# dgrzech/ir-sgmcmc

Hardware: AMD Instinct MI355X
Metric: SG-MCMC transitions/sec (full _SGLD_transition) (higher is better)
Workload: dtype f32; 1 GPU; 256^3 synthetic pair, SVF_3D 12 steps, GMM(K=4)/LCC(s=1) + virtual decimation, RegLoss_L2 w=1.4, Sobolev s=3, uniform noise 0.1, SGLD lr 0.4, Philox noise; init=identity, chains=1, parallelism=1 independent chain(s)

## Files before the change

include/irsgmcmc.h:

```cpp
#ifndef IRSGMCMC_H
#define IRSGMCMC_H

#include <stddef.h>
#include <stdint.h>

#ifdef __cplusplus
extern "C" {
#endif
#pragma GCC visibility push(default)

#define IRS_MAX_COMPONENTS 8
#define IRS_MAX_CHAINS 8
#define IRS_MAX_HALF_WIDTH 4
#define IRS_MAX_LABELS 64
#define IRS_HAUSDORFF_MAX_PERCENTILES 4

enum { IRS_DATA_GMM_LCC = 0, IRS_DATA_SSD = 1 };
enum { IRS_REG_L2 = 0, IRS_REG_LOGNORMAL = 1, IRS_REG_STUDENT = 2, IRS_REG_LOGNORMAL_L2 = 3 };


int irs_perturb_smooth(const float* v, const float* sigma, const float* eps, float tau, const float* kernel, int s,
                       int C, int D, int H, int W, float* tmp, float* out, uint64_t seed, uint64_t iteration,
                       void* stream);

// ... 306 lines not shown
int irs_set_fixed(irs_ctx* ctx, const float* fixed_im, int fixed_chains, void* stream);
int irs_get_state(irs_ctx* ctx, irs_state* out, void* stream);
int irs_set_state(irs_ctx* ctx, const irs_state* in, void* stream);
int irs_get_scalars(irs_ctx* ctx, irs_scalars* out, void* stream);

int irs_gmm_init(irs_ctx* ctx, const irs_io* io, const float* v_sample, int warm_up, void* stream);

int irs_transition(irs_ctx* ctx, const irs_io* io, void* stream);

int irs_flush(irs_ctx* ctx, void* stream);
int irs_recovered_transitions(const irs_ctx* ctx, uint64_t* out);
int irs_sparse_adjoint_set(irs_ctx* ctx, int on);
int irs_sparse_adjoint_get(irs_ctx* ctx, int32_t* out, void* stream);
int irs_sparse_data_set(irs_ctx* ctx, int on);
int irs_sparse_data_get(irs_ctx* ctx, int32_t* out, void* stream);

typedef struct irs_timings {
    float total_ms;
    float exp_fwd_ms;
    float exp_bwd_kernel_ms;
    float exp_bwd_total_ms;
    float smooth_ms;
    float data_ms;
    float update_ms;
    float exp_bwd_primary_avg_ms;
} irs_timings;
int irs_transition_timed(irs_ctx* ctx, const irs_io* io, void* stream, irs_timings* out);

typedef struct irs_comm irs_comm;
#define IRS_COMM_ID_BYTES 128
// ... 95 lines not shown
```

ir_sgmcmc_amd/_lib.py:

```python
import ctypes as C
import os

import torch

_HERE = os.path.dirname(os.path.abspath(__file__))
LIB_PATH = os.environ.get('IRS_LIB') or os.path.join(_HERE, 'csrc', 'libirsgmcmc.so')

IRS_MAX_COMPONENTS = 8
IRS_MAX_CHAINS = 8
IRS_MAX_HALF_WIDTH = 4
IRS_MAX_LABELS = 64
IRS_HAUSDORFF_MAX_PERCENTILES = 4
IRS_LABEL_BINS = 10
IRS_JACOBIAN_SUMMARY_INTS, IRS_JACOBIAN_SUMMARY_FLOATS = 4, 5
IRS_JACOBIAN_WS_BYTES = 1024 * (IRS_JACOBIAN_SUMMARY_INTS + IRS_JACOBIAN_SUMMARY_FLOATS) * 8
IRS_COVARIANCE_SUMMARY_INTS, IRS_COVARIANCE_SUMMARY_FLOATS = 2, 8
IRS_COVARIANCE_WS_BYTES = 1024 * (IRS_COVARIANCE_SUMMARY_INTS + IRS_COVARIANCE_SUMMARY_FLOATS) * 8
IRS_COMPARE_SUMMARY_INTS, IRS_COMPARE_SUMMARY_FLOATS = 4, 13
IRS_COMPARE_WS_BYTES = 1024 * (IRS_COMPARE_SUMMARY_INTS + IRS_COMPARE_SUMMARY_FLOATS) * 8
IRS_QUANTILE_MIN_BINS, IRS_QUANTILE_MAX_BINS, IRS_QUANTILE_MAX_PROBS, IRS_QUANTILE_MAX_RECORDS = 4, 256, 8, 65535
IRS_QUANTILE_SUMMARY_INTS, IRS_QUANTILE_SUMMARY_FLOATS = 3, 5
IRS_QUANTILE_WS_BYTES = 1024 * (IRS_QUANTILE_SUMMARY_INTS + IRS_QUANTILE_SUMMARY_FLOATS) * 8
IRS_ICE_SUMMARY_INTS, IRS_ICE_SUMMARY_FLOATS = 2, 3
IRS_ICE_WS_BYTES = IRS_MAX_CHAINS * 1024 * (IRS_ICE_SUMMARY_INTS + IRS_ICE_SUMMARY_FLOATS) * 8
# ... 195 lines not shown
    'irs_destroy': [_P],
    'irs_workspace_bytes': [_P],
    'irs_velocity_dims': [_P, C.POINTER(C.c_int32 * 3)],
    'irs_set_fixed': [_P, _P, _I, _P],
    'irs_get_state': [_P, C.POINTER(IrsState), _P],
    'irs_set_state': [_P, C.POINTER(IrsState), _P],
    'irs_get_scalars': [_P, C.POINTER(IrsScalars), _P],
    'irs_gmm_init': [_P, C.POINTER(IrsIO), _P, _I, _P],
    'irs_transition': [_P, C.POINTER(IrsIO), _P],
    'irs_flush': [_P, _P],
    'irs_recovered_transitions': [_P, C.POINTER(C.c_uint64)],
    'irs_sparse_adjoint_set': [_P, _I],
    'irs_sparse_adjoint_get': [_P, _I32P, _P],
    'irs_sparse_data_set': [_P, _I],
    'irs_sparse_data_get': [_P, _I32P, _P],
    'irs_transition_timed': [_P, C.POINTER(IrsIO), _P, C.POINTER(IrsTimings)],
    'irs_comm_unique_id': [C.POINTER(C.c_uint8 * IRS_COMM_ID_BYTES)],
    'irs_comm_create_rccl': [C.POINTER(C.c_uint8 * IRS_COMM_ID_BYTES), _I, _I, C.POINTER(_P)],
    'irs_comm_create_ipc': [C.c_char_p, _I, _I, C.POINTER(_P)],
    'irs_comm_create_callbacks': [EXCHANGE_FN, ALLREDUCE_FN, _P, _I, _I, C.POINTER(_P)],
    'irs_comm_destroy': [_P],
    'irs_comm_probe': [_P, C.c_size_t, C.c_size_t, _I, _P, C.POINTER(C.c_double * 2)],
    'irs_comm_describe': [_P, C.c_char_p, C.c_size_t],
    'irs_comm_rank': [_P],
    'irs_comm_world': [_P],
    'irs_comm_selftest': [_P, _P],
    'irs_slab_plan_layout': [C.POINTER(IrsConfig), C.POINTER(IrsSlabConfig), _I, _I, C.POINTER(IrsSlabLayout)],
    'irs_slab_create': [C.POINTER(IrsConfig), C.POINTER(IrsSlabConfig), _P, C.POINTER(_P)],
    'irs_slab_get_layout': [_P, C.POINTER(IrsSlabLayout)],
    'irs_slab_transition': [_P, C.POINTER(IrsIO), _P],
# ... 65 lines not shown
```

ir_sgmcmc_amd/csrc/adjoint_plan.hip:

```cpp
#include "adjoint_plan.h"

#include "kernels.h"

namespace irs {

constexpr int kExtChunk = 32;

template <typename T>
__device__ __forceinline__ void extent_body(const T* __restrict__ g, int* __restrict__ ext, const Vol& vol) {
    const int x = (int)blockIdx.x * 64 + ((int)threadIdx.x & 63), y = (int)blockIdx.y * 4 + ((int)threadIdx.x >> 6);
    const int nch = (vol.D + kExtChunk - 1) / kExtChunk;
    const int chain = (int)blockIdx.z / nch, za = ((int)blockIdx.z - chain * nch) * kExtChunk, zb = min(za + kExtChunk, vol.D);
    if (x >= vol.W || y >= vol.H) return;
    const int64_t plane = (int64_t)vol.H * vol.W;
    const T* __restrict__ p = g + (int64_t)chain * vol.V + (int64_t)y * vol.W + x;
    int lo = vol.D, hi = -1;
#pragma unroll 8
    for (int z = za; z < zb; ++z) {
        const bool nz = p[z * plane] != (T)0;
        lo = nz ? min(lo, z) : lo;
        hi = nz ? z : hi;
    }
    if (hi < 0) return;
    int* e = ext + ((int64_t)chain * plane + (int64_t)y * vol.W + x) * 2;
    atomicMax(e, vol.D - lo);
    atomicMax(e + 1, hi + 1);
}
__global__ __launch_bounds__(kBlock) void grad_extent_kernel(const float* __restrict__ g, int* __restrict__ ext, Vol vol) {
    extent_body<float>(g, ext, vol);
}
__global__ __launch_bounds__(kBlock) void mask_extent_kernel(const uint8_t* __restrict__ mask, int* __restrict__ ext, Vol vol) {
    extent_body<uint8_t>(mask, ext, vol);
}
static void launch_extent(const float* g, const uint8_t* mask, int* ext, int chains, Vol vol, hipStream_t st) {
    (void)hipMemsetAsync(ext, 0, sizeof(int) * 2 * (size_t)chains * vol.H * vol.W, st);
    const int nch = (vol.D + kExtChunk - 1) / kExtChunk;
    const dim3 grid((unsigned)((vol.W + 63) / 64), (unsigned)((vol.H + 3) / 4), (unsigned)(nch * chains));
    if (g) hipLaunchKernelGGL(grad_extent_kernel, grid, dim3(kBlock), 0, st, g, ext, vol);
    else hipLaunchKernelGGL(mask_extent_kernel, grid, dim3(kBlock), 0, st, mask, ext, vol);
}

__device__ __forceinline__ bool chain_is_dense(const unsigned* __restrict__ dmax, int chain, int C, int no_steps) {
    bool dense = false;
    if (!dmax) return false;
    for (int k = 0; k < no_steps; ++k) {
        const unsigned* b = dmax + ((int64_t)k * C + chain) * 4;
        const float m = fmaxf(fmaxf(__uint_as_float(b[0]), __uint_as_float(b[1])), __uint_as_float(b[2]));
        dense |= !(m < 1.0f);
    }
    return dense;
}

__global__ __launch_bounds__(kWave) void plan_runs_kernel(const int* __restrict__ ext, int ext_chains, const unsigned* __restrict__ dmax,
                                                          int* __restrict__ runs, Vol vol, int C, int no_steps, int ntx, int nty,
                                                          PlanShape shape) {
// ... 118 lines not shown
        count[2 * k] = min(base, cap);
        count[2 * k + 1] = min(s_nrun, cap);
    }
    if (tid < C) {
        int* s = stats + ((int64_t)k * C + tid) * kPlanStats;
        s[0] = chain_is_dense(dmax, tid, C, no_steps) ? 0 : 1;
        s[1] = L;
        s[2] = s_pieces[tid];
        s[3] = s_planes[tid];
    }
}

static size_t plan_align(size_t b) { return (b + 255) / 256 * 256; }

struct PlanLayout {
    size_t ext, runs, colplan, entries, count, stats, total;
    int cap, ntx, nty;
};
static PlanLayout plan_layout(Vol vol, int C, int no_steps) {
    PlanLayout l;
    l.ntx = (vol.W + kPlanTX - 1) / kPlanTX;
    l.nty = (vol.H + kPlanTY - 1) / kPlanTY;
    const size_t cols = (size_t)C * l.ntx * l.nty;
    l.cap = plan_entries_cap((int)cols, vol.D);
    size_t off = 0;
    auto take = [&](size_t bytes) { const size_t o = off; off += plan_align(bytes); return o; };
    l.ext = take(sizeof(int) * 2 * (size_t)C * vol.H * vol.W);
    l.runs = take(sizeof(int) * 2 * cols * no_steps);
    l.colplan = take(sizeof(ColPlan) * cols * no_steps);
    l.entries = take(sizeof(PlanEntry) * (size_t)l.cap * no_steps);
    l.count = take(sizeof(int) * 2 * no_steps);
    l.stats = take(sizeof(int) * kPlanStats * (size_t)C * no_steps);
    l.total = off;
    return l;
}

size_t adjoint_plan_bytes(Vol vol, int C, int no_steps) { return plan_layout(vol, C, no_steps).total; }

AdjointPlan adjoint_plan_views(char* base, Vol vol, int C, int no_steps) {
    const PlanLayout l = plan_layout(vol, C, no_steps);
    AdjointPlan p;
    p.ext = (int*)(base + l.ext);
    p.runs = (int*)(base + l.runs);
    p.colplan = (ColPlan*)(base + l.colplan);
    p.entries = (PlanEntry*)(base + l.entries);
    p.count = (int*)(base + l.count);
    p.stats = (int*)(base + l.stats);
    p.cap = l.cap;
    p.ntx = l.ntx;
    p.nty = l.nty;
    return p;
}

void launch_adjoint_plan(const float* g_warped, const unsigned* dmax, const AdjointPlan& plan, int no_steps, int C, Vol vol,
                         int64_t G, int forced_len, hipStream_t st) {
    const int g = (int)(G > 0 ? G : 1024);
    const PlanShape shape{kPlanTX, kPlanTY, no_steps, 1, {kFillNext, kFillNext}, {g, g}, kPlanMinLen};
    launch_extent(g_warped, nullptr, plan.ext, C, vol, st);
    hipLaunchKernelGGL(plan_runs_kernel, dim3((unsigned)(C * plan.ntx * plan.nty), (unsigned)no_steps), dim3(kWave), 0, st, plan.ext, C, dmax,
                       plan.runs, vol, C, no_steps, plan.ntx, plan.nty, shape);
    hipLaunchKernelGGL(plan_lists_kernel, dim3((unsigned)no_steps), dim3(kPlanBlock), 0, st, plan.runs, dmax, plan.colplan, plan.entries, plan.count,
                       plan.stats, vol, C, no_steps, plan.ntx, plan.nty, plan.cap, shape, forced_len);
}

struct DataLayout {
    size_t ext, runs, hull, colplan, entries, count, stats, nll, total;
    int cap, ntx, nty, wtx, wty;
};
static DataLayout data_layout(Vol vol, int C) {
    DataLayout l;
    l.ntx = (vol.W + kLccTX - 1) / kLccTX;
    l.nty = (vol.H + kLccTY - 1) / kLccTY;
    l.wtx = (vol.W + kWarpTX - 1) / kWarpTX;
    l.wty = (vol.H + kWarpTY - 1) / kWarpTY;
// ... 31 lines not shown
    p.nty = l.nty;
    p.wtx = l.wtx;
    p.wty = l.wty;
    return p;
}

static int data_list_resident(int s, bool bwd, int C) {
    const int64_t res = lcc_plan_resident(s, bwd, bwd && C > 1);
    return (int)(res > 0 ? res : 1024);
}
int data_plan_run_bound(const DataPlan& plan, int s, bool bwd, int C, Vol vol) {
    return plan_run_bound(C * plan.ntx * plan.nty, vol.D, data_list_resident(s, bwd, C), plan.forced_len);
}

void launch_data_plan(const uint8_t* mask, int mask_chains, const DataPlan& plan, int s, bool lists, int C, Vol vol, hipStream_t st) {
    launch_extent(nullptr, mask, plan.ext, mask_chains, vol, st);
    const PlanShape warp{kWarpTX, kWarpTY, 3 * s, 0, {kFillNone, kFillNone}, {1, 1}, kPlanMinLen};
    hipLaunchKernelGGL(plan_runs_kernel, dim3((unsigned)(C * plan.wtx * plan.wty), 1u), dim3(kWave), 0, st, plan.ext, mask_chains, nullptr,
                       plan.hull, vol, C, 1, plan.wtx, plan.wty, warp);
    if (!lists) return;
    const PlanShape lcc{kLccTX, kLccTY, 2 * s, s, {kFillAll, kFillNone}, {data_list_resident(s, true, C), data_list_resident(s, false, C)},
                        kPlanMinLen};
    hipLaunchKernelGGL(plan_runs_kernel, dim3((unsigned)(C * plan.ntx * plan.nty), 2u), dim3(kWave), 0, st, plan.ext, mask_chains, nullptr,
                       plan.runs, vol, C, 2, plan.ntx, plan.nty, lcc);
    hipLaunchKernelGGL(plan_lists_kernel, dim3(2u), dim3(kPlanBlock), 0, st, plan.runs, nullptr, plan.colplan, plan.entries, plan.count, plan.stats,
                       vol, C, 2, plan.ntx, plan.nty, plan.cap, lcc, plan.forced_len);
}

}
```

ir_sgmcmc_amd/csrc/api_ctx.hip:

```cpp
#include <math.h>
#include <string.h>

#include <new>

#include "adjoint_plan.h"
#include "api_checks.h"
#include "comm.h"

using namespace irs;

static size_t align_up(size_t x) { return (x + 255) & ~(size_t)255; }

static bool is_capturing(hipStream_t st) {
    hipStreamCaptureStatus cap = hipStreamCaptureStatusNone;
    (void)hipStreamIsCapturing(st, &cap);
    return cap != hipStreamCaptureStatusNone;
}


int irs::create_ctx(const irs_config* cfg, const SlabInfo* sl, irs_ctx** out) {
    if (!cfg || !out) return fail("irs_create: null argument");
    const int D = cfg->dims[0], H = cfg->dims[1], W = cfg->dims[2], C = cfg->no_chains;
    if (!dims_ok(C, D, H, W) || !chain_count_ok(C)) return fail("irs_create: bad dims / chains (C <= %d)", IRS_MAX_CHAINS);
    if (cfg->no_steps < 1 || cfg->no_steps > 30) return fail("irs_create: no_steps out of range");
// ... 7 lines not shown
    if ((cfg->reg_loss == IRS_REG_STUDENT || cfg->reg_loss == IRS_REG_LOGNORMAL_L2) && cfg->reg_learnable)
        return fail("irs_create: RegLoss_Student / RegLoss_LogNormal_L2 have no learnable parameters");
    if (cfg->reg_loss == IRS_REG_STUDENT && !(cfg->w_reg_prior_rate > 0.0 && cfg->w_reg_prior_shape > 0.0))
        return fail("irs_create: RegLoss_Student needs a0 > 0 and b0 > 0 (w_reg_prior_shape / w_reg_prior_rate)");
    const bool any_cps = cfg->cps[0] || cfg->cps[1] || cfg->cps[2];
    if (any_cps && (cfg->cps[0] < 1 || cfg->cps[1] < 1 || cfg->cps[2] < 1 || cfg->cps[0] > 8 || cfg->cps[1] > 8 || cfg->cps[2] > 8))
        return fail("irs_create: control point spacing must be 1..8 on every axis");

    irs_ctx* c = new (std::nothrow) irs_ctx();
    if (!c) return fail("irs_create: out of host memory");
    memset((void*)c, 0, sizeof(*c));
    context_born();
    c->kn = global_knobs();
    c->sparse_adjoint = true;
    c->sparse_data = 1;
    c->cfg = *cfg;
    c->C = C;
    c->vol = make_vol(D, H, W);
    if (sl && sl->on) {
        c->sl = *sl;
        c->vol.V = (int64_t)(sl->hi - sl->lo) * H * W;
    }
    c->ffd = any_cps;
    c->volv = c->ffd ? make_vol(control_points(D, cfg->cps[0]), control_points(H, cfg->cps[1]), control_points(W, cfg->cps[2]))
                     : c->vol;
    c->sob.s = cfg->sobolev_s;
    for (int i = 0; i <= 2 * cfg->sobolev_s; ++i) c->sob.k[i] = cfg->sobolev_kernel[i];
    if (c->ffd)
        for (int a = 0; a < 3; ++a) c->spl[a] = make_spline(cfg->cps[a]);

// ... 101 lines not shown
    init.ssd_inv_sigma = cfg->data_loss == IRS_DATA_SSD ? 1.0f / cfg->ssd_sigma : 0.0f;
    if (cfg->reg_loss == IRS_REG_L2 || cfg->reg_loss == IRS_REG_LOGNORMAL_L2) init.st.reg_param[0] = log((double)cfg->w_reg);
    for (int ch = 0; ch < IRS_MAX_CHAINS; ++ch) init.sc.alpha[ch] = 1.0;
    hipError_t e = hipMemcpy(c->state, &init, sizeof(init), hipMemcpyHostToDevice);
    if (e == hipSuccess) {
        launch_refresh_derived(c->state, c->dcfg, nullptr);
        e = hipDeviceSynchronize();
    }
    for (int i = 0; i < 8 && e == hipSuccess; ++i) e = hipEventCreate(&c->ev[i]);
    for (int i = 0; i < 64 && e == hipSuccess; ++i) e = hipEventCreate(&c->ev_bwd[i]);
    for (int i = 0; i < 4 && e == hipSuccess; ++i) e = hipEventCreateWithFlags(&c->ra_ev[i], hipEventDisableTiming);
    if (c->C > 1 && !c->sl.on && c->kn.chain_overlap) {
        if (e == hipSuccess) e = hipStreamCreateWithFlags(&c->side, hipStreamNonBlocking);
        for (int i = 0; i < 2 * c->C && e == hipSuccess; ++i) e = hipEventCreateWithFlags(&c->ev_side[i], hipEventDisableTiming);
    }
    if (e == hipSuccess) e = hipHostMalloc((void**)&c->hint, sizeof(unsigned) * kHintWords, hipHostMallocDefault);
    if (e == hipSuccess)
        for (int i = 0; i < kHintWords; ++i) c->hint[i] = i < kHintWords - 8 ? 0x7f800000u : 0u;
    if (e != hipSuccess) {
        irs_destroy(c);
        return fail("irs_create: state initialisation failed: %s", hipGetErrorString(e));
    }
    *out = c;
    return 0;
}

int irs::check_io(const irs_ctx* c, const irs_io* io, const char* who) {
    if (!c || !io) return fail("%s: null argument", who);
    if (!io->fixed_im || !io->moving_im || !io->mask) return fail("%s: fixed_im, moving_im and mask are required", who);
    if (!broadcast_ok(io->fixed_chains, c->C) || !broadcast_ok(io->moving_chains, c->C) || !broadcast_ok(io->mask_chains, c->C))
// ... 7 lines not shown
int irs_create(const irs_config* cfg, irs_ctx** out) { return irs::create_ctx(cfg, nullptr, out); }

void irs_destroy(irs_ctx* c) {
    if (!c) return;
    (void)hipDeviceSynchronize();
    if (c->sl.on) slab_release(c);
    for (int i = 0; i < 8; ++i)
        if (c->ev[i]) (void)hipEventDestroy(c->ev[i]);
    for (int i = 0; i < 64; ++i)
        if (c->ev_bwd[i]) (void)hipEventDestroy(c->ev_bwd[i]);
    for (int i = 0; i < 4; ++i)
        if (c->ra_ev[i]) (void)hipEventDestroy(c->ra_ev[i]);
    for (int i = 0; i < 2 * IRS_MAX_CHAINS; ++i)
        if (c->ev_side[i]) (void)hipEventDestroy(c->ev_side[i]);
    if (c->side) (void)hipStreamDestroy(c->side);
    if (c->lin.dev) (void)hipFree(c->lin.dev);
    if (c->hint) (void)hipHostFree(c->hint);
    if (c->slab) (void)hipFree(c->slab);
    delete c;
    context_gone();
}

size_t irs_workspace_bytes(const irs_ctx* c) { return c ? c->slab_bytes : 0; }

int irs_velocity_dims(const irs_ctx* c, int32_t out[3]) {
    if (!c || !out) return fail("irs_velocity_dims: null argument");
    out[0] = c->volv.D;
    out[1] = c->volv.H;
    out[2] = c->volv.W;
    return 0;
// ... 45 lines not shown
    HIP_TRY(hipMemcpyAsync(&c->state->st, in, sizeof(irs_state), hipMemcpyHostToDevice, (hipStream_t)stream));
    launch_refresh_derived(c->state, c->dcfg, (hipStream_t)stream);
    LAUNCH_CHECK();
    HIP_TRY(hipStreamSynchronize((hipStream_t)stream));
    return 0;
}

int irs_get_scalars(irs_ctx* c, irs_scalars* out, void* stream) {
    if (!c || !out) return fail("irs_get_scalars: null argument");
    if (flush_or_failed_transport(c, stream)) return 1;
    HIP_TRY(hipMemcpyAsync(out, &c->state->sc, sizeof(irs_scalars), hipMemcpyDeviceToHost, (hipStream_t)stream));
    HIP_TRY(hipStreamSynchronize((hipStream_t)stream));
    return 0;
}

static int forward_pass(irs_ctx* c, const irs_io* io, const float* v, bool with_noise, bool with_jitter, float* vs,
                        float* warped, float* z, float* gradm, int chains, hipStream_t st, int timed, int data_on = 0) {
    const irs_config& cfg = c->cfg;
    const int C = chains;
    const uint64_t* it = &c->state->st.iteration;
    if (!c->dmax_clean) HIP_TRY(hipMemsetAsync(c->dmax, 0, sizeof(unsigned) * 4 * c->C * (cfg.no_steps + 1), st));
    c->dmax_clean = false;
    bool have_dmax0 = false;
    const float amp = (float)sqrt(2.0 * (double)cfg.lr);
    if (with_noise && cfg.sobolev_s > 0 && !c->ffd && c->kn.fuse_noise && !(io->sigma && io->eps)) {
        have_dmax0 = true;
        launch_perturb_sobolev_march(v, io->sigma, io->eps, amp, vs, c->sob, C, c->volv, c->dmax, cfg.no_steps, cfg.seed, 0, it, st);
    } else {
        float* first = cfg.sobolev_s > 0 ? c->tmpA : vs;
        if (with_noise) launch_perturb(v, io->sigma, io->eps, amp, first, C, c->volv, cfg.seed, 0, it, st);
        else HIP_TRY(hipMemcpyAsync(first, v, (size_t)C * 3 * c->volv.V * sizeof(float), hipMemcpyDeviceToDevice, st));
        if (cfg.sobolev_s > 0) {
// ... 6 lines not shown
        const int G[3] = {c->volv.D, c->volv.H, c->volv.W};
        ffd_up(vs, c->dense, c->tmpA, C, c->vol, G, c->spl, st);
        dense = c->dense;
    }
    if (timed) HIP_TRY(hipEventRecord(c->ev[1], st));
    const int64_t field = (int64_t)c->C * 3 * c->vol.V;
    const Lin lin = c->lin.lin();
    if (!have_dmax0) launch_field_absmax(dense, true, cfg.no_steps, c->dmax, C, c->vol, st);
    for (int k = 0; k < cfg.no_steps; ++k) {
        const float* in = k == 0 ? dense : c->steps + (int64_t)(k - 1) * field;
        float* out = c->steps + (int64_t)k * field;
        launch_exp_step_fwd_march(in, out, k == 0, cfg.no_steps, C, c->vol, lin, c->dmax + (int64_t)k * c->C * 4,
                                  c->dmax + (int64_t)(k + 1) * c->C * 4, predicted_small(c, k), fwd_lay(c, k), st);
    }
    if (timed) HIP_TRY(hipEventRecord(c->ev[2], st));
    const float* d_last = c->steps + (int64_t)(cfg.no_steps - 1) * field;
    const float alpha = with_jitter ? cfg.uniform_alpha : 0.0f;
    launch_warp_fwd(io->moving_im, io->moving_chains == 1 ? 0 : c->vol.V, d_last, io->unif, alpha, warped, gradm, 1, C, c->vol, lin,
                    cfg.seed, 0, it, st, data_on > 0 ? c->dplan.hull : nullptr);
    if (cfg.data_loss == IRS_DATA_GMM_LCC && data_on > 1)
        launch_lcc_fwd_plan(c->fhat, c->fhat_chains == 1 ? 0 : c->vol.V, warped, z, c->sigM, cfg.lcc_s, C, c->vol, c->dplan, st);
    else if (cfg.data_loss == IRS_DATA_GMM_LCC)
        launch_lcc_fwd_march(c->fhat, c->fhat_chains == 1 ? 0 : c->vol.V, warped, z, c->sigM, cfg.lcc_s, C, c->vol, st);
    else
        launch_residual_ssd(io->fixed_im, io->fixed_chains == 1 ? 0 : c->vol.V, warped, z, C, c->vol, st);
    LAUNCH_CHECK();
    return 0;
}

int irs_gmm_init(irs_ctx* c, const irs_io* io, const float* v_sample, int warm_up, void* stream) {
    if (check_io(c, io, "irs_gmm_init")) return 1;
    if (c->cfg.data_loss != IRS_DATA_GMM_LCC) return 0;
    hipStream_t st = (hipStream_t)stream;
    const size_t bytes = (size_t)3 * c->volv.V * sizeof(float);
    if (v_sample) HIP_TRY(hipMemcpyAsync(c->tmpB, v_sample, bytes, hipMemcpyDeviceToDevice, st));
    else HIP_TRY(hipMemsetAsync(c->tmpB, 0, bytes, st));
    if (forward_pass(c, io, c->tmpB, false, false, c->vs, c->warped, c->z, nullptr, 1, st, 0)) return 1;
    launch_masked_moments(c->z, io->mask, c->stat_partials, c->vol, st);
    launch_gmm_init_from_moments(c->state, c->stat_partials, stats_blocks(c->vol), c->dcfg, st);
    launch_stats(c->cfg.virtual_decimation, c->z, io->mask, c->state, c->stat_partials, c->vol, st, c->dcfg.K);
    launch_chain_scalar(c->state, c->stat_partials, stats_blocks(c->vol), 0, 1, c->dcfg, st);
    for (int i = 0; i < warm_up; ++i) {
        launch_stats(0, c->z, io->mask, c->state, c->stat_partials, c->vol, st, c->dcfg.K);
        launch_chain_scalar(c->state, c->stat_partials, stats_blocks(c->vol), 0, 2, c->dcfg, st);
    }
    LAUNCH_CHECK();
    return 0;
}

static int enqueue_transition(irs_ctx* c, const irs_io* io, hipStream_t st, int timed, bool no_assumptions) {

    const irs_config& cfg = c->cfg;
    const int C = c->C;
    const Vol vol = c->vol, volv = c->volv;
    const Lin lin = c->lin.lin();
    float* vs = io->curr_state ? io->curr_state : c->vs;
    float* warped = io->im_moving_warped ? io->im_moving_warped : c->warped;
    float* z = io->residuals ? io->residuals : c->z;
    const uint64_t* it = &c->state->st.iteration;
    const int saved_mode = c->kn.predict_variants;
    if (no_assumptions) c->kn.predict_variants = 0;
// ... 10 lines not shown
    vd.n = cfg.no_steps;
    vd.C = C;
    for (int k = 0; k < cfg.no_steps && k < 32; ++k) {
        skip_any[k] = predicted_below(c, k, global_knobs().lds_from <= 2 ? 0.75f : 1.5f);
        skip_r2[k] = skip_any[k] && predicted_tiny(c, k);
        if (skip_r2[k]) vd.need_lt1 |= 1u << k;
        else if (skip_any[k]) (global_knobs().lds_from > 2 ? vd.need_lt2 : vd.need_lt1) |= 1u << k;
    }

    if (timed) HIP_TRY(hipEventRecord(c->ev[0], st));
    const bool fuse_warp_bwd = c->kn.fuse_warp_bwd != 0;
    const bool lcc = cfg.data_loss == IRS_DATA_GMM_LCC;
    const int forced_piece = c->sparse_data > 1 ? c->sparse_data : 0;
    int data_on = 0;
    c->dplan.forced_len = forced_piece;
    if (c->sparse_data && c->dplan.entries && !io->im_moving_warped && !io->residuals &&
        (forced_piece > 0 || plan_min(lcc_dense_seg_len(vol, C, false), lcc_dense_seg_len(vol, c->nll_seg_C, true)) > kPlanMinLen)) {
        const bool one_launch = C == 1 || (c->kn.data_batch != 0 && !(c->side && c->kn.chain_overlap != 0));
        data_on = !lcc ? 1 : one_launch ? 3 : 2;
        launch_data_plan(io->mask, io->mask_chains, c->dplan, lcc ? cfg.lcc_s : 0, lcc, C, vol, st);
    }
    c->data_on = data_on;
    if (forward_pass(c, io, io->v, true, cfg.uniform_alpha > 0.0f, vs, warped, z, fuse_warp_bwd ? c->gA : nullptr, C, st, timed, data_on)) return 1;
    const int64_t field = (int64_t)C * 3 * vol.V;
    const float* d_last = c->steps + (int64_t)(cfg.no_steps - 1) * field;
    if (io->transformation || io->displacement) launch_svf_outputs(d_last, io->transformation, io->displacement, C, vol, lin, st);

    const int upd_blocks = sgld_update_blocks_per_chain(volv, C);
    const bool energy_in_update = (cfg.reg_loss == IRS_REG_L2 || cfg.reg_loss == IRS_REG_LOGNORMAL_L2) &&
                                  (int64_t)upd_blocks * C <= (int64_t)kMaxPartialBlocks * IRS_MAX_CHAINS &&
                                  c->kn.energy_in_update != 0;
    if (!energy_in_update) {
        launch_reg_energy(vs, c->energy_partials, C, volv, st);
        launch_reg_scalar(c->state, c->energy_partials, energy_blocks(volv), c->dcfg, st, vd);
    }

    const int sb = stats_blocks(vol);
    const bool overlap = C > 1 && c->side && c->kn.chain_overlap != 0;
// ... 13 lines not shown
            ds = c->side;
        }
        launch_data_bwd(cfg.data_loss, f, 0, zc, c->sigM + (int64_t)ch * vol.V, mask, 0, nullptr, c->state, ch,
                        c->gM + (int64_t)ch * vol.V, c->nll_partials + (int64_t)ch * c->nll_blocks, cfg.lcc_s, 1, vol, ds, c->nll_seg_C);
        if (ds != st) HIP_TRY(hipEventRecord(c->ev_side[2 * ch + 1], c->side));
    }
    if (data_on == 3)
        launch_lcc_data_bwd_plan(c->fhat, c->fhat_chains == 1 ? 0 : vol.V, z, c->sigM, io->mask, io->mask_chains == 1 ? 0 : vol.V, c->state, c->gM,
                                 cfg.lcc_s, C, vol, c->dplan, st);
    else if (batch)
        launch_data_bwd(cfg.data_loss, c->fhat, c->fhat_chains == 1 ? 0 : vol.V, z, c->sigM, io->mask, io->mask_chains == 1 ? 0 : vol.V, nullptr,
                        c->state, 0, c->gM, c->nll_partials, cfg.lcc_s, C, vol, st, c->nll_seg_C);
    if (!fuse_warp_bwd)
        launch_warp_bwd(io->moving_im, io->moving_chains == 1 ? 0 : vol.V, d_last, io->unif,
                        cfg.uniform_alpha > 0.0f ? cfg.uniform_alpha : 0.0f, c->gM, c->gA, C, vol, lin, cfg.seed, 0, it, st);
    const bool sparse = c->sparse_adjoint && c->plan.entries != nullptr &&
                        (global_knobs().march_seg > 0 || exp_bwd_dense_seg_len(vol, C) > kPlanMinLen);
    c->plan_on = sparse;
    if (sparse) launch_adjoint_plan(c->gM, c->dmax, c->plan, cfg.no_steps, C, vol, exp_bwd_plan_resident(), global_knobs().march_seg, st);
    LAUNCH_CHECK();
    if (timed) HIP_TRY(hipEventRecord(c->ev[3], st));
    const float* dense = c->ffd ? c->dense : vs;
    float* g0 = nullptr;
    {
        const float* G = c->gA;
        float* bufs[2] = {c->gB, c->gA};
        int cur = 0;
        for (int k = cfg.no_steps - 1; k >= 0; --k) {
            float* out = bufs[cur];
            const float* dk = k == 0 ? dense : c->steps + (int64_t)(k - 1) * field;
            if (timed) HIP_TRY(hipEventRecord(c->ev_bwd[2 * k], st));
            const unsigned* dm = c->dmax + (int64_t)k * C * 4;
            const float* gscale = fuse_warp_bwd && k == cfg.no_steps - 1 ? c->gM : nullptr;
            const int lay = bwd_lay(c, k) | (gscale ? 2 : 0);
// ... 104 lines not shown
    c->sparse_adjoint = on != 0;
    return 0;
}

int irs_sparse_adjoint_get(irs_ctx* c, int32_t* out, void* stream) {
    if (!c || !out) return fail("irs_sparse_adjoint_get: null argument");
    const size_t n = (size_t)c->cfg.no_steps * c->C * kPlanStats;
    memset(out, 0, n * sizeof(int32_t));
    if (!c->plan.stats || !c->plan_on || c->n_enqueued == 0) return 0;
    if (irs_flush(c, stream)) return 1;
    HIP_TRY(hipMemcpyAsync(out, c->plan.stats, n * sizeof(int32_t), hipMemcpyDeviceToHost, (hipStream_t)stream));
    HIP_TRY(hipStreamSynchronize((hipStream_t)stream));
    return 0;
}

int irs_sparse_data_set(irs_ctx* c, int on) {
    if (!c) return fail("irs_sparse_data_set: null argument");
    if (on < 0) return fail("irs_sparse_data_set: 0 (off), 1 (on) or a piece length");
    c->sparse_data = on;
    return 0;
}

int irs_sparse_data_get(irs_ctx* c, int32_t* out, void* stream) {
    if (!c || !out) return fail("irs_sparse_data_get: null argument");
    const int C = c->C;
    memset(out, 0, (size_t)kDataKernels * C * kPlanStats * sizeof(int32_t));
    if (!c->dplan.entries || c->data_on == 0 || c->n_enqueued == 0) return 0;
    if (irs_flush(c, stream)) return 1;
    const size_t tiles = (size_t)c->dplan.wtx * c->dplan.wty;
    int* hull = (int*)malloc(sizeof(int) * 2 * tiles * C);
// ... 46 lines not shown
```

ir_sgmcmc_amd/csrc/ctx.h:

```cpp
#pragma once
#include <stdlib.h>
#include <string.h>

#include "kernels.h"
#include "scalar_kernels.h"

struct irs_comm;

namespace irs {

int fail(const char* fmt, ...);

#define HIP_TRY(expr)                                                                               \
    do {                                                                                            \
        hipError_t e_ = (expr);                                                                     \
        if (e_ != hipSuccess) return irs::fail("%s failed: %s", #expr, hipGetErrorString(e_));      \
    } while (0)

#define LAUNCH_CHECK()                                                                              \
    do {                                                                                            \
        hipError_t e_ = hipGetLastError();                                                          \
        if (e_ != hipSuccess) return irs::fail("kernel launch failed: %s", hipGetErrorString(e_)); \
    } while (0)

// ... 20 lines not shown
    irs::LinTables lin;
    irs::Taps sob;
    irs::SplineTaps spl[3];
    char* slab;
    size_t slab_bytes;
    float *steps, *tmpA, *tmpB, *vs, *gA, *gB, *gC, *warped, *z, *sigM, *fhat, *gM, *dense;
    double *stat_partials, *energy_partials, *nll_partials;
    double *stat_sum, *energy_sum, *nll_sum;
    unsigned* dmax;
    irs::AdjointPlan plan;
    bool sparse_adjoint = true;
    bool plan_on = false;
    irs::DataPlan dplan;
    int sparse_data = 1;
    int data_on = 0;
    float* cmm;
    unsigned* hint = nullptr;
    irs::DevState* state;
    int fhat_chains;
    bool fixed_set;
    int nll_blocks;
    int nll_seg_C;
    hipEvent_t ev[8];
    hipEvent_t ev_bwd[64];
    hipEvent_t ra_ev[4];
    hipStream_t side = nullptr;
    hipEvent_t ev_side[2 * IRS_MAX_CHAINS] = {};
    uint64_t n_enqueued = 0;
    irs::Knobs kn;
    bool dmax_clean = false;
// ... 119 lines not shown
```

ir_sgmcmc_amd/csrc/kernels.h:

```cpp
#pragma once
#include "common.h"

namespace irs {

struct Taps {
    float k[2 * IRS_MAX_HALF_WIDTH + 1];
    int s;
};

struct SplineTaps {
    float k[32];
    int cps;
};

struct LinTables {
    float* dev = nullptr;
    int D = 0, H = 0, W = 0;
    Lin lin() const { return Lin{dev, dev + W, dev + W + H}; }
};
int ensure_lin_tables(LinTables& t, int D, int H, int W, hipStream_t st);
int cached_lin(int D, int H, int W, hipStream_t st, Lin* out);

void launch_perturb(const float* v, const float* sigma, const float* eps, float amp, float* out, int C, Vol vol,
                    uint64_t seed, uint64_t iteration, const uint64_t* dev_iteration, hipStream_t st);
// ... 19 lines not shown
                               const unsigned* dmax_in, unsigned* dmax_out, bool only_r1, int lay, hipStream_t st);
struct AdjointPlan;
void launch_exp_step_bwd_march(const float* G, const float* dk, float* gout, bool prescale, int no_steps, int C, Vol vol,
                               Lin lin, const unsigned* dmax, int max_radius, bool r2_owns_rest, const float* gscale, int lay,
                               hipEvent_t after_primary, hipStream_t st, const AdjointPlan* plan = nullptr, int step = 0);
int exp_bwd_dense_seg_len(Vol vol, int C);
int64_t exp_bwd_plan_resident();
size_t coarse_minmax_bytes(Vol vol, int C);
void launch_exp_step_bwd_lds(const float* G, const float* dk, float* gout, bool prescale, int no_steps, int C, Vol vol,
                             Lin lin, const unsigned* dmax, int halo, int gather_radius, const float* gscale, int lay,
                             float* cmm, hipStream_t st);
void launch_field_absmax(const float* d, bool prescale, int no_steps, unsigned* dmax, int C, Vol vol, hipStream_t st);

struct PlanEntry;
struct ColPlan;
struct AdjointPlan {
    int* ext = nullptr;
    int* runs = nullptr;
    ColPlan* colplan = nullptr;
    PlanEntry* entries = nullptr;
    int* count = nullptr;
    int* stats = nullptr;
    int cap = 0, ntx = 0, nty = 0;
};
size_t adjoint_plan_bytes(Vol vol, int C, int no_steps);
AdjointPlan adjoint_plan_views(char* base, Vol vol, int C, int no_steps);
void launch_adjoint_plan(const float* g_warped, const unsigned* dmax, const AdjointPlan& plan, int no_steps, int C, Vol vol,
                         int64_t G, int forced_len, hipStream_t st);
struct DataPlan {
    int* ext = nullptr;
    int* runs = nullptr;
    int* hull = nullptr;
    ColPlan* colplan = nullptr;
    PlanEntry* entries = nullptr;
    int* count = nullptr;
    int* stats = nullptr;
    double* nll = nullptr;
    int cap = 0, ntx = 0, nty = 0, wtx = 0, wty = 0;
    int forced_len = 0;
};
size_t data_plan_bytes(Vol vol, int C);
DataPlan data_plan_views(char* base, Vol vol, int C);
// ... 249 lines not shown
```

ir_sgmcmc_amd/engine.py:

```python
import ctypes as C
import math
from dataclasses import dataclass, field
from typing import Optional, Sequence, Tuple

import torch
from scipy.special import digamma

from . import _lib as L
from .ops import control_grid_size, sobolev_kernel_1d


@dataclass
class EngineConfig:
    dims: Tuple[int, int, int]
    no_chains: int = 1
    cps: Optional[Tuple[int, int, int]] = None
    no_steps: int = 12
    sobolev_s: int = 3
    sobolev_lambda: float = 0.5
    lr: float = 0.4
    uniform_noise: float = 0.1
    virtual_decimation: bool = True
    data_loss: str = 'GMM'
    gmm_components: int = 4
# ... 132 lines not shown
        keys = ('engaged', 'piece_len', 'pieces', 'run_planes')
        return [[dict(zip(keys, buf[(k * ch + c) * 4:(k * ch + c) * 4 + 4])) for c in range(ch)] for k in range(n)]

    def set_sparse_data(self, on):
        L.check(self.lib.irs_sparse_data_set(self._ctx, int(on)))

    @_on_device
    def sparse_data(self):
        ch = self.cfg.no_chains
        buf = (C.c_int32 * (4 * ch * 4))()
        L.check(self.lib.irs_sparse_data_get(self._ctx, buf, self._stream()))
        keys = ('engaged', 'piece_len', 'pieces', 'run_planes')
        return {name: [dict(zip(keys, buf[(k * ch + c) * 4:(k * ch + c) * 4 + 4])) for c in range(ch)]
                for k, name in enumerate(('warp', 'map', 'stats', 'data_term'))}

    @property
    def workspace_bytes(self):
        return int(self.lib.irs_workspace_bytes(self._ctx))

    @_on_device
    def state(self):
        st = L.IrsState()
        L.check(self.lib.irs_get_state(self._ctx, C.byref(st), self._stream()))
        return st

    @_on_device
    def set_state(self, st):
        L.check(self.lib.irs_set_state(self._ctx, C.byref(st), self._stream()))

    @_on_device
# ... 52 lines not shown
```

Before: 258.2 transitions/s.

## Build adjoint plan from mask extent and optionally overlap planning on side stream

The sparse adjoint plan now derives its z-extent from the mask, dilated by the LCC window, instead of scanning the warped-image gradient after the data term. This lets the plan be built right after the forward SVF steps rather than on the critical path after warp backward. An optional high-priority side stream, off by default, can run the data and adjoint planning concurrently with the forward steps. The memset is replaced by a clear kernel and the ext buffer is shared with the data plan. The mask-derived extent is more conservative than the gradient extent, so the adjoint may march over more voxels.

Result: no change. 259.2 transitions/s (median of 4 runs) (+0.4%).

```diff
diff --git a/include/irsgmcmc.h b/include/irsgmcmc.h
--- a/include/irsgmcmc.h
+++ b/include/irsgmcmc.h
@@ -344,6 +344,8 @@
 int irs_sparse_adjoint_get(irs_ctx* ctx, int32_t* out, void* stream);
 int irs_sparse_data_set(irs_ctx* ctx, int on);
 int irs_sparse_data_get(irs_ctx* ctx, int32_t* out, void* stream);
+int irs_plan_stream_set(irs_ctx* ctx, int on);
+int irs_plan_stream_get(const irs_ctx* ctx, int32_t* out);
 
 typedef struct irs_timings {
     float total_ms;
diff --git a/ir_sgmcmc_amd/_lib.py b/ir_sgmcmc_amd/_lib.py
--- a/ir_sgmcmc_amd/_lib.py
+++ b/ir_sgmcmc_amd/_lib.py
@@ -233,6 +233,8 @@
     'irs_sparse_adjoint_get': [_P, _I32P, _P],
     'irs_sparse_data_set': [_P, _I],
     'irs_sparse_data_get': [_P, _I32P, _P],
+    'irs_plan_stream_set': [_P, _I],
+    'irs_plan_stream_get': [_P, _I32P],
     'irs_transition_timed': [_P, C.POINTER(IrsIO), _P, C.POINTER(IrsTimings)],
     'irs_comm_unique_id': [C.POINTER(C.c_uint8 * IRS_COMM_ID_BYTES)],
     'irs_comm_create_rccl': [C.POINTER(C.c_uint8 * IRS_COMM_ID_BYTES), _I, _I, C.POINTER(_P)],
diff --git a/ir_sgmcmc_amd/csrc/adjoint_plan.hip b/ir_sgmcmc_amd/csrc/adjoint_plan.hip
--- a/ir_sgmcmc_amd/csrc/adjoint_plan.hip
+++ b/ir_sgmcmc_amd/csrc/adjoint_plan.hip
@@ -7,13 +7,13 @@
 constexpr int kExtChunk = 32;
 
 template <typename T>
-__device__ __forceinline__ void extent_body(const T* __restrict__ g, int* __restrict__ ext, const Vol& vol) {
+__device__ __forceinline__ void extent_body(const T* __restrict__ mask, int* __restrict__ ext, const Vol& vol) {
     const int x = (int)blockIdx.x * 64 + ((int)threadIdx.x & 63), y = (int)blockIdx.y * 4 + ((int)threadIdx.x >> 6);
     const int nch = (vol.D + kExtChunk - 1) / kExtChunk;
     const int chain = (int)blockIdx.z / nch, za = ((int)blockIdx.z - chain * nch) * kExtChunk, zb = min(za + kExtChunk, vol.D);
     if (x >= vol.W || y >= vol.H) return;
     const int64_t plane = (int64_t)vol.H * vol.W;
-    const T* __restrict__ p = g + (int64_t)chain * vol.V + (int64_t)y * vol.W + x;
+    const T* __restrict__ p = mask + (int64_t)chain * vol.V + (int64_t)y * vol.W + x;
     int lo = vol.D, hi = -1;
 #pragma unroll 8
     for (int z = za; z < zb; ++z) {
@@ -26,19 +26,26 @@
     atomicMax(e, vol.D - lo);
     atomicMax(e + 1, hi + 1);
 }
+__global__ __launch_bounds__(kBlock) void mask_extent_kernel(const uint8_t* __restrict__ mask, int* __restrict__ ext, Vol vol) {
+    extent_body<uint8_t>(mask, ext, vol);
+}
 __global__ __launch_bounds__(kBlock) void grad_extent_kernel(const float* __restrict__ g, int* __restrict__ ext, Vol vol) {
     extent_body<float>(g, ext, vol);
 }
-__global__ __launch_bounds__(kBlock) void mask_extent_kernel(const uint8_t* __restrict__ mask, int* __restrict__ ext, Vol vol) {
-    extent_body<uint8_t>(mask, ext, vol);
-}
-static void launch_extent(const float* g, const uint8_t* mask, int* ext, int chains, Vol vol, hipStream_t st) {
-    (void)hipMemsetAsync(ext, 0, sizeof(int) * 2 * (size_t)chains * vol.H * vol.W, st);
+__global__ __launch_bounds__(kBlock) void ext_clear_kernel(int2* __restrict__ ext, int n) {
+    const int i = (int)blockIdx.x * kBlock + (int)threadIdx.x;
+    if (i < n) ext[i] = make_int2(0, 0);
+}
+static void launch_extent(const uint8_t* mask, const float* g, int chains, int* ext, Vol vol, hipStream_t st) {
+    const int n_ext = chains * vol.H * vol.W;
+    hipLaunchKernelGGL(ext_clear_kernel, dim3((unsigned)((n_ext + kBlock - 1) / kBlock)), dim3(kBlock), 0, st, (int2*)ext, n_ext);
     const int nch = (vol.D + kExtChunk - 1) / kExtChunk;
     const dim3 grid((unsigned)((vol.W + 63) / 64), (unsigned)((vol.H + 3) / 4), (unsigned)(nch * chains));
     if (g) hipLaunchKernelGGL(grad_extent_kernel, grid, dim3(kBlock), 0, st, g, ext, vol);
     else hipLaunchKernelGGL(mask_extent_kernel, grid, dim3(kBlock), 0, st, mask, ext, vol);
 }
+void launch_mask_extent(const uint8_t* mask, int mask_chains, int* ext, Vol vol, hipStream_t st) { launch_extent(mask, nullptr, mask_chains, ext, vol, st); }
+void launch_grad_extent(const float* g_warped, int C, int* ext, Vol vol, hipStream_t st) { launch_extent(nullptr, g_warped, C, ext, vol, st); }
 
 __device__ __forceinline__ bool chain_is_dense(const unsigned* __restrict__ dmax, int chain, int C, int no_steps) {
     bool dense = false;
@@ -187,7 +194,7 @@
 static size_t plan_align(size_t b) { return (b + 255) / 256 * 256; }
 
 struct PlanLayout {
-    size_t ext, runs, colplan, entries, count, stats, total;
+    size_t runs, colplan, entries, count, stats, total;
     int cap, ntx, nty;
 };
 static PlanLayout plan_layout(Vol vol, int C, int no_steps) {
@@ -198,7 +205,6 @@
     l.cap = plan_entries_cap((int)cols, vol.D);
     size_t off = 0;
     auto take = [&](size_t bytes) { const size_t o = off; off += plan_align(bytes); return o; };
-    l.ext = take(sizeof(int) * 2 * (size_t)C * vol.H * vol.W);
     l.runs = take(sizeof(int) * 2 * cols * no_steps);
     l.colplan = take(sizeof(ColPlan) * cols * no_steps);
     l.entries = take(sizeof(PlanEntry) * (size_t)l.cap * no_steps);
@@ -213,7 +219,6 @@
 AdjointPlan adjoint_plan_views(char* base, Vol vol, int C, int no_steps) {
     const PlanLayout l = plan_layout(vol, C, no_steps);
     AdjointPlan p;
-    p.ext = (int*)(base + l.ext);
     p.runs = (int*)(base + l.runs);
     p.colplan = (ColPlan*)(base + l.colplan);
     p.entries = (PlanEntry*)(base + l.entries);
@@ -225,12 +230,11 @@
     return p;
 }
 
-void launch_adjoint_plan(const float* g_warped, const unsigned* dmax, const AdjointPlan& plan, int no_steps, int C, Vol vol,
+void launch_adjoint_plan(const int* ext, int ext_chains, const unsigned* dmax, const AdjointPlan& plan, int no_steps, int beyond, int C, Vol vol,
                          int64_t G, int forced_len, hipStream_t st) {
     const int g = (int)(G > 0 ? G : 1024);
-    const PlanShape shape{kPlanTX, kPlanTY, no_steps, 1, {kFillNext, kFillNext}, {g, g}, kPlanMinLen};
-    launch_extent(g_warped, nullptr, plan.ext, C, vol, st);
-    hipLaunchKernelGGL(plan_runs_kernel, dim3((unsigned)(C * plan.ntx * plan.nty), (unsigned)no_steps), dim3(kWave), 0, st, plan.ext, C, dmax,
+    const PlanShape shape{kPlanTX, kPlanTY, no_steps + beyond, 1, {kFillNext, kFillNext}, {g, g}, kPlanMinLen};
+    hipLaunchKernelGGL(plan_runs_kernel, dim3((unsigned)(C * plan.ntx * plan.nty), (unsigned)no_steps), dim3(kWave), 0, st, ext, ext_chains, dmax,
                        plan.runs, vol, C, no_steps, plan.ntx, plan.nty, shape);
     hipLaunchKernelGGL(plan_lists_kernel, dim3((unsigned)no_steps), dim3(kPlanBlock), 0, st, plan.runs, dmax, plan.colplan, plan.entries, plan.count,
                        plan.stats, vol, C, no_steps, plan.ntx, plan.nty, plan.cap, shape, forced_len);
@@ -292,7 +296,7 @@
 }
 
 void launch_data_plan(const uint8_t* mask, int mask_chains, const DataPlan& plan, int s, bool lists, int C, Vol vol, hipStream_t st) {
-    launch_extent(nullptr, mask, plan.ext, mask_chains, vol, st);
+    launch_mask_extent(mask, mask_chains, plan.ext, vol, st);
     const PlanShape warp{kWarpTX, kWarpTY, 3 * s, 0, {kFillNone, kFillNone}, {1, 1}, kPlanMinLen};
     hipLaunchKernelGGL(plan_runs_kernel, dim3((unsigned)(C * plan.wtx * plan.wty), 1u), dim3(kWave), 0, st, plan.ext, mask_chains, nullptr,
                        plan.hull, vol, C, 1, plan.wtx, plan.wty, warp);
diff --git a/ir_sgmcmc_amd/csrc/api_ctx.hip b/ir_sgmcmc_amd/csrc/api_ctx.hip
--- a/ir_sgmcmc_amd/csrc/api_ctx.hip
+++ b/ir_sgmcmc_amd/csrc/api_ctx.hip
@@ -45,6 +45,7 @@
     c->kn = global_knobs();
     c->sparse_adjoint = true;
     c->sparse_data = 1;
+    c->plan_stream = false;
     c->cfg = *cfg;
     c->C = C;
     c->vol = make_vol(D, H, W);
@@ -176,6 +177,12 @@
         if (e == hipSuccess) e = hipStreamCreateWithFlags(&c->side, hipStreamNonBlocking);
         for (int i = 0; i < 2 * c->C && e == hipSuccess; ++i) e = hipEventCreateWithFlags(&c->ev_side[i], hipEventDisableTiming);
     }
+    if (planned) {
+        int prio_least = 0, prio_greatest = 0;
+        (void)hipDeviceGetStreamPriorityRange(&prio_least, &prio_greatest);
+        if (e == hipSuccess) e = hipStreamCreateWithPriority(&c->plan_st, hipStreamNonBlocking, prio_greatest);
+        for (int i = 0; i < 4 && e == hipSuccess; ++i) e = hipEventCreateWithFlags(&c->ev_plan[i], hipEventDisableTiming);
+    }
     if (e == hipSuccess) e = hipHostMalloc((void**)&c->hint, sizeof(unsigned) * kHintWords, hipHostMallocDefault);
     if (e == hipSuccess)
         for (int i = 0; i < kHintWords; ++i) c->hint[i] = i < kHintWords - 8 ? 0x7f800000u : 0u;
@@ -213,6 +220,9 @@
     for (int i = 0; i < 2 * IRS_MAX_CHAINS; ++i)
         if (c->ev_side[i]) (void)hipEventDestroy(c->ev_side[i]);
     if (c->side) (void)hipStreamDestroy(c->side);
+    for (int i = 0; i < 4; ++i)
+        if (c->ev_plan[i]) (void)hipEventDestroy(c->ev_plan[i]);
+    if (c->plan_st) (void)hipStreamDestroy(c->plan_st);
     if (c->lin.dev) (void)hipFree(c->lin.dev);
     if (c->hint) (void)hipHostFree(c->hint);
     if (c->slab) (void)hipFree(c->slab);
@@ -288,8 +298,7 @@
     return 0;
 }
 
-static int forward_pass(irs_ctx* c, const irs_io* io, const float* v, bool with_noise, bool with_jitter, float* vs,
-                        float* warped, float* z, float* gradm, int chains, hipStream_t st, int timed, int data_on = 0) {
+static int forward_steps(irs_ctx* c, const irs_io* io, const float* v, bool with_noise, float* vs, int chains, hipStream_t st, int timed) {
     const irs_config& cfg = c->cfg;
     const int C = chains;
     const uint64_t* it = &c->state->st.iteration;
@@ -326,7 +335,17 @@
                                   c->dmax + (int64_t)(k + 1) * c->C * 4, predicted_small(c, k), fwd_lay(c, k), st);
     }
     if (timed) HIP_TRY(hipEventRecord(c->ev[2], st));
-    const float* d_last = c->steps + (int64_t)(cfg.no_steps - 1) * field;
+    LAUNCH_CHECK();
+    return 0;
+}
+
+static int forward_data(irs_ctx* c, const irs_io* io, bool with_jitter, float* warped, float* z, float* gradm, int chains, hipStream_t st,
+                        int data_on = 0) {
+    const irs_config& cfg = c->cfg;
+    const int C = chains;
+    const uint64_t* it = &c->state->st.iteration;
+    const Lin lin = c->lin.lin();
+    const float* d_last = c->steps + (int64_t)(cfg.no_steps - 1) * (int64_t)c->C * 3 * c->vol.V;
     const float alpha = with_jitter ? cfg.uniform_alpha : 0.0f;
     launch_warp_fwd(io->moving_im, io->moving_chains == 1 ? 0 : c->vol.V, d_last, io->unif, alpha, warped, gradm, 1, C, c->vol, lin,
                     cfg.seed, 0, it, st, data_on > 0 ? c->dplan.hull : nullptr);
@@ -347,7 +366,7 @@
     const size_t bytes = (size_t)3 * c->volv.V * sizeof(float);
     if (v_sample) HIP_TRY(hipMemcpyAsync(c->tmpB, v_sample, bytes, hipMemcpyDeviceToDevice, st));
     else HIP_TRY(hipMemsetAsync(c->tmpB, 0, bytes, st));
-    if (forward_pass(c, io, c->tmpB, false, false, c->vs, c->warped, c->z, nullptr, 1, st, 0)) return 1;
+    if (forward_steps(c, io, c->tmpB, false, c->vs, 1, st, 0) || forward_data(c, io, false, c->warped, c->z, nullptr, 1, st)) return 1;
     launch_masked_moments(c->z, io->mask, c->stat_partials, c->vol, st);
     launch_gmm_init_from_moments(c->state, c->stat_partials, stats_blocks(c->vol), c->dcfg, st);
     launch_stats(c->cfg.virtual_decimation, c->z, io->mask, c->state, c->stat_partials, c->vol, st, c->dcfg.K);
@@ -357,6 +376,23 @@
         launch_chain_scalar(c->state, c->stat_partials, stats_blocks(c->vol), 0, 2, c->dcfg, st);
     }
     LAUNCH_CHECK();
+    return 0;
+}
+
+static int plan_fork(irs_ctx* c, int group, hipStream_t st, hipStream_t* ps) {
+    *ps = st;
+    if (!c->plan_stream || !c->plan_st || is_capturing(st)) return 0;
+    HIP_TRY(hipEventRecord(c->ev_plan[2 * group], st));
+    HIP_TRY(hipStreamWaitEvent(c->plan_st, c->ev_plan[2 * group], 0));
+    *ps = c->plan_st;
+    return 0;
+}
+static int plan_done(irs_ctx* c, int group, hipStream_t st, hipStream_t ps) {
+    if (ps != st) HIP_TRY(hipEventRecord(c->ev_plan[2 * group + 1], ps));
+    return 0;
+}
+static int plan_join(irs_ctx* c, int group, hipStream_t st, hipStream_t ps) {
+    if (ps != st) HIP_TRY(hipStreamWaitEvent(st, c->ev_plan[2 * group + 1], 0));
     return 0;
 }
 
@@ -397,14 +433,33 @@
     const int forced_piece = c->sparse_data > 1 ? c->sparse_data : 0;
     int data_on = 0;
     c->dplan.forced_len = forced_piece;
+    const bool sparse = c->sparse_adjoint && c->plan.entries != nullptr &&
+                        (global_knobs().march_seg > 0 || exp_bwd_dense_seg_len(vol, C) > kPlanMinLen);
+    c->plan_on = sparse;
+    hipStream_t psA = st, psB = st;
+    bool from_mask = false;
     if (c->sparse_data && c->dplan.entries && !io->im_moving_warped && !io->residuals &&
         (forced_piece > 0 || plan_min(lcc_dense_seg_len(vol, C, false), lcc_dense_seg_len(vol, c->nll_seg_C, true)) > kPlanMinLen)) {
         const bool one_launch = C == 1 || (c->kn.data_batch != 0 && !(c->side && c->kn.chain_overlap != 0));
         data_on = !lcc ? 1 : one_launch ? 3 : 2;
-        launch_data_plan(io->mask, io->mask_chains, c->dplan, lcc ? cfg.lcc_s : 0, lcc, C, vol, st);
     }
     c->data_on = data_on;
-    if (forward_pass(c, io, io->v, true, cfg.uniform_alpha > 0.0f, vs, warped, z, fuse_warp_bwd ? c->gA : nullptr, C, st, timed, data_on)) return 1;
+    from_mask = sparse && (data_on == 3 || !lcc);
+    if (data_on || from_mask) {
+        if (plan_fork(c, 0, st, &psA)) return 1;
+        if (data_on) launch_data_plan(io->mask, io->mask_chains, c->dplan, lcc ? cfg.lcc_s : 0, lcc, C, vol, psA);
+        else launch_mask_extent(io->mask, io->mask_chains, c->dplan.ext, vol, psA);
+        if (plan_done(c, 0, st, psA)) return 1;
+    }
+    if (forward_steps(c, io, io->v, true, vs, C, st, timed)) return 1;
+    if (from_mask) {
+        if (plan_fork(c, 1, st, &psB)) return 1;
+        launch_adjoint_plan(c->dplan.ext, io->mask_chains, c->dmax, c->plan, cfg.no_steps, lcc ? 2 * cfg.lcc_s : 0, C, vol, exp_bwd_plan_resident(),
+                            global_knobs().march_seg, psB);
+        if (plan_done(c, 1, st, psB)) return 1;
+    }
+    if (plan_join(c, 0, st, psA)) return 1;
+    if (forward_data(c, io, cfg.uniform_alpha > 0.0f, warped, z, fuse_warp_bwd ? c->gA : nullptr, C, st, data_on)) return 1;
     const int64_t field = (int64_t)C * 3 * vol.V;
     const float* d_last = c->steps + (int64_t)(cfg.no_steps - 1) * field;
     if (io->transformation || io->displacement) launch_svf_outputs(d_last, io->transformation, io->displacement, C, vol, lin, st);
@@ -448,10 +503,11 @@
     if (!fuse_warp_bwd)
         launch_warp_bwd(io->moving_im, io->moving_chains == 1 ? 0 : vol.V, d_last, io->unif,
                         cfg.uniform_alpha > 0.0f ? cfg.uniform_alpha : 0.0f, c->gM, c->gA, C, vol, lin, cfg.seed, 0, it, st);
-    const bool sparse = c->sparse_adjoint && c->plan.entries != nullptr &&
-                        (global_knobs().march_seg > 0 || exp_bwd_dense_seg_len(vol, C) > kPlanMinLen);
-    c->plan_on = sparse;
-    if (sparse) launch_adjoint_plan(c->gM, c->dmax, c->plan, cfg.no_steps, C, vol, exp_bwd_plan_resident(), global_knobs().march_seg, st);
+    if (plan_join(c, 1, st, psB)) return 1;
+    if (sparse && !from_mask) {
+        launch_grad_extent(c->gM, C, c->dplan.ext, vol, st);
+        launch_adjoint_plan(c->dplan.ext, C, c->dmax, c->plan, cfg.no_steps, 0, C, vol, exp_bwd_plan_resident(), global_knobs().march_seg, st);
+    }
     LAUNCH_CHECK();
     if (timed) HIP_TRY(hipEventRecord(c->ev[3], st));
     const float* dense = c->ffd ? c->dense : vs;
@@ -586,6 +642,18 @@
     return 0;
 }
 
+int irs_plan_stream_set(irs_ctx* c, int on) {
+    if (!c) return fail("irs_plan_stream_set: null argument");
+    c->plan_stream = on != 0;
+    return 0;
+}
+
+int irs_plan_stream_get(const irs_ctx* c, int32_t* out) {
+    if (!c || !out) return fail("irs_plan_stream_get: null argument");
+    *out = c->plan_stream && c->plan_st ? 1 : 0;
+    return 0;
+}
+
 int irs_sparse_data_set(irs_ctx* c, int on) {
     if (!c) return fail("irs_sparse_data_set: null argument");
     if (on < 0) return fail("irs_sparse_data_set: 0 (off), 1 (on) or a piece length");
diff --git a/ir_sgmcmc_amd/csrc/ctx.h b/ir_sgmcmc_amd/csrc/ctx.h
--- a/ir_sgmcmc_amd/csrc/ctx.h
+++ b/ir_sgmcmc_amd/csrc/ctx.h
@@ -58,6 +58,9 @@
     irs::DataPlan dplan;
     int sparse_data = 1;
     int data_on = 0;
+    hipStream_t plan_st = nullptr;
+    hipEvent_t ev_plan[4] = {};
+    bool plan_stream = false;
     float* cmm;
     unsigned* hint = nullptr;
     irs::DevState* state;
diff --git a/ir_sgmcmc_amd/csrc/kernels.h b/ir_sgmcmc_amd/csrc/kernels.h
--- a/ir_sgmcmc_amd/csrc/kernels.h
+++ b/ir_sgmcmc_amd/csrc/kernels.h
@@ -57,8 +57,9 @@
 
 struct PlanEntry;
 struct ColPlan;
+void launch_mask_extent(const uint8_t* mask, int mask_chains, int* ext, Vol vol, hipStream_t st);
+void launch_grad_extent(const float* g_warped, int C, int* ext, Vol vol, hipStream_t st);
 struct AdjointPlan {
-    int* ext = nullptr;
     int* runs = nullptr;
     ColPlan* colplan = nullptr;
     PlanEntry* entries = nullptr;
@@ -68,7 +69,7 @@
 };
 size_t adjoint_plan_bytes(Vol vol, int C, int no_steps);
 AdjointPlan adjoint_plan_views(char* base, Vol vol, int C, int no_steps);
-void launch_adjoint_plan(const float* g_warped, const unsigned* dmax, const AdjointPlan& plan, int no_steps, int C, Vol vol,
+void launch_adjoint_plan(const int* ext, int ext_chains, const unsigned* dmax, const AdjointPlan& plan, int no_steps, int beyond, int C, Vol vol,
                          int64_t G, int forced_len, hipStream_t st);
 struct DataPlan {
     int* ext = nullptr;
diff --git a/ir_sgmcmc_amd/engine.py b/ir_sgmcmc_amd/engine.py
--- a/ir_sgmcmc_amd/engine.py
+++ b/ir_sgmcmc_amd/engine.py
@@ -170,6 +170,15 @@
         return {name: [dict(zip(keys, buf[(k * ch + c) * 4:(k * ch + c) * 4 + 4])) for c in range(ch)]
                 for k, name in enumerate(('warp', 'map', 'stats', 'data_term'))}
 
+    def set_plan_stream(self, on):
+        L.check(self.lib.irs_plan_stream_set(self._ctx, int(bool(on))))
+
+    @property
+    def plan_stream(self):
+        on = C.c_int32()
+        L.check(self.lib.irs_plan_stream_get(self._ctx, C.byref(on)))
+        return bool(on.value)
+
     @property
     def workspace_bytes(self):
         return int(self.lib.irs_workspace_bytes(self._ctx))
```
